# jczarnowski/DeepFactors

Hardware: NVIDIA H100
Metric: keyframe-pair Jacobian+JtJ evals/sec (640x480, C=32) (higher is better)
Workload: dtype f32

## Files before the change

### deepfactors_b200/csrc/dfk_window.cu

```cuda
#include <cuda_runtime.h>
#include <stdint.h>

#include "dfk_internal.h"

namespace dfk {

namespace {

__device__ __forceinline__ int packed_index(int i, int j, int NP) { return i * NP - (i * (i - 1)) / 2 + (j - i); }
__device__ __forceinline__ float rec_h(const float* rec, int a, int b, int NP)
{
  return a <= b ? rec[packed_index(a, b, NP)] : rec[packed_index(b, a, NP)];
}

__device__ __forceinline__ int link_row0(int r) { return r < 6 ? r : 6 + r; }
__device__ __forceinline__ int link_row1(int r, int C) { return r < 6 ? 6 + r : 6 + C + r; }

__global__ void __launch_bounds__(256)
window_assemble_kernel(WindowDev w, const float* __restrict__ records, const float* __restrict__ geo,
                       float* __restrict__ out)
{
  const int C = w.code_size, B = 6 + C, NP = 12 + C;
  const int NH = NP * (NP + 1) / 2, REC = NH + NP + 2;
  const int NG = 12 + 2 * C, NHG = NG * (NG + 1) / 2, RECG = NHG + NG + 2;
  float* tail = out + (size_t)w.num_keyframes * (B * B + B) + (size_t)w.num_pairs * B * 6;
  const int job = blockIdx.x;
  if (job < w.num_keyframes) {
    const int k = job;
    float* D = out + (size_t)k * B * B;
    float* g = out + (size_t)w.num_keyframes * B * B + (size_t)k * B;
    const int a0 = w.kf0_ptr[k], a1 = w.kf0_ptr[k + 1];
    const int b0 = w.kf1_ptr[k], b1 = w.kf1_ptr[k + 1];
    const int l00 = w.lk0_ptr[k], l01 = w.lk0_ptr[k + 1];
    const int l10 = w.lk1_ptr[k], l11 = w.lk1_ptr[k + 1];
    for (int e = threadIdx.x; e < B * B + B; e += blockDim.x) {
      float s = 0.0f;
      if (e < B * B) {
        const int r = e / B, c = e - r * B;
        const int lr = r < 6 ? r : 6 + r, lc = c < 6 ? c : 6 + c;
        for (int q = a0; q < a1; ++q) s += rec_h(records + (size_t)w.kf0_items[q] * REC, lr, lc, NP);
        if (r < 6 && c < 6)
          for (int q = b0; q < b1; ++q) s += rec_h(records + (size_t)w.kf1_items[q] * REC, 6 + r, 6 + c, NP);
        for (int q = l00; q < l01; ++q) s += rec_h(geo + (size_t)w.lk0_links[q] * RECG, link_row0(r), link_row0(c), NG);
        for (int q = l10; q < l11; ++q)
          s += rec_h(geo + (size_t)w.lk1_links[q] * RECG, link_row1(r, C), link_row1(c, C), NG);
        D[e] = s;
      } else {
        const int r = e - B * B;
        const int lr = r < 6 ? r : 6 + r;
        for (int q = a0; q < a1; ++q) s -= records[(size_t)w.kf0_items[q] * REC + NH + lr];
        if (r < 6)
          for (int q = b0; q < b1; ++q) s -= records[(size_t)w.kf1_items[q] * REC + NH + 6 + r];
        for (int q = l00; q < l01; ++q) s -= geo[(size_t)w.lk0_links[q] * RECG + NHG + link_row0(r)];
        for (int q = l10; q < l11; ++q) s -= geo[(size_t)w.lk1_links[q] * RECG + NHG + link_row1(r, C)];
        g[r] = s;
      }
    }
  } else if (job < w.num_keyframes + w.num_pairs) {
    const int p = job - w.num_keyframes;
    float* O = out + (size_t)w.num_keyframes * (B * B + B) + (size_t)p * B * 6;
    const int i0 = w.pair_ptr[p], i1 = w.pair_ptr[p + 1];
    for (int e = threadIdx.x; e < B * 6; e += blockDim.x) {
      const int r = e / 6, c = e - r * 6;
      const int lr = r < 6 ? r : 6 + r;
      float s = 0.0f;
      for (int q = i0; q < i1; ++q) s += rec_h(records + (size_t)w.pair_items[q] * REC, lr, 6 + c, NP);
      O[e] = s;
    }
  } else if (job < w.num_keyframes + w.num_pairs + w.num_links) {
    const int l = job - w.num_keyframes - w.num_pairs;
    float* O = tail + 2 + (size_t)l * B * B;
    const float* rec = geo + (size_t)l * RECG;
    for (int e = threadIdx.x; e < B * B; e += blockDim.x) {
      const int r = e / B, c = e - r * B;
      O[e] = rec_h(rec, link_row0(r), link_row1(c, C), NG);
    }
  } else {
    __shared__ float red_f[8], red_i[8];
    float f = 0.0f, ni = 0.0f;
    for (int i = threadIdx.x; i < w.num_items; i += blockDim.x) {
      const float* rec = records + (size_t)i * REC;
      const uint32_t inl = __float_as_uint(rec[NH + NP + 1]);
      if (w.item_area[i] == 0.0f) {
        f += rec[NH + NP];
      } else {
        if (inl > 0) f += rec[NH + NP] / (float)inl * w.item_area[i];
        ni += (float)inl;
      }
    }
    for (int l = threadIdx.x; l < w.num_links; l += blockDim.x) f += geo[(size_t)l * RECG + NHG + NG];
    for (int o = 16; o > 0; o >>= 1) {
      f += __shfl_xor_sync(0xffffffffu, f, o);
      ni += __shfl_xor_sync(0xffffffffu, ni, o);
    }
    if ((threadIdx.x & 31) == 0) {
      red_f[threadIdx.x >> 5] = f;
      red_i[threadIdx.x >> 5] = ni;
    }
    __syncthreads();
    if (threadIdx.x == 0) {
      float sf = 0.0f, si = 0.0f;
      for (int k = 0; k < (int)(blockDim.x >> 5); ++k) {
        sf += red_f[k];
        si += red_i[k];
      }
      tail[0] = sf;
      tail[1] = si;
    }
  }
}

}

cudaError_t launch_window_assemble(const WindowDev& w, const float* records_dev, const float* geo_records_dev,
                                   float* out_dev, cudaStream_t stream)
{
  window_assemble_kernel<<<w.num_keyframes + w.num_pairs + w.num_links + 1, 256, 0, stream>>>(w, records_dev,
                                                                                             geo_records_dev, out_dev);
  return cudaGetLastError();
}

}
```

Before: 32190.

## Split window assembly across more blocks, unroll gathers, enable programmatic dependent launch

Each keyframe, pair and link job is now spread over several blocks so every thread computes exactly one output element, instead of one block looping over all elements. The gather loops are unrolled by four so index and record loads can be issued in parallel. The kernel is launched with programmatic stream serialization and calls cudaGridDependencySynchronize, which lets its launch overlap the tail of the previous kernel. This adds blocks and some index arithmetic, and it relies on PDL support.

```diff
diff --git a/deepfactors_b200/csrc/dfk_window.cu b/deepfactors_b200/csrc/dfk_window.cu
--- a/deepfactors_b200/csrc/dfk_window.cu
+++ b/deepfactors_b200/csrc/dfk_window.cu
@@ -8,75 +8,90 @@
 namespace {
 
 __device__ __forceinline__ int packed_index(int i, int j, int NP) { return i * NP - (i * (i - 1)) / 2 + (j - i); }
-__device__ __forceinline__ float rec_h(const float* rec, int a, int b, int NP)
-{
-  return a <= b ? rec[packed_index(a, b, NP)] : rec[packed_index(b, a, NP)];
-}
 
 __device__ __forceinline__ int link_row0(int r) { return r < 6 ? r : 6 + r; }
 __device__ __forceinline__ int link_row1(int r, int C) { return r < 6 ? 6 + r : 6 + C + r; }
 
-__global__ void __launch_bounds__(256)
+constexpr int kWinThreads = 256;
+constexpr int kWinUnroll = 4;
+
+template <bool SUB>
+__device__ __forceinline__ float gather(float s, const float* __restrict__ base, size_t stride, int off,
+                                        const int* __restrict__ idx, int q0, int q1)
+{
+  for (int q = q0; q < q1; q += kWinUnroll) {
+    int id[kWinUnroll];
+#pragma unroll
+    for (int u = 0; u < kWinUnroll; ++u) id[u] = q + u < q1 ? idx[q + u] : 0;
+    float v[kWinUnroll];
+#pragma unroll
+    for (int u = 0; u < kWinUnroll; ++u) v[u] = q + u < q1 ? base[(size_t)id[u] * stride + off] : 0.0f;
+#pragma unroll
+    for (int u = 0; u < kWinUnroll; ++u)
+      if (q + u < q1) s = SUB ? s - v[u] : s + v[u];
+  }
+  return s;
+}
+
+__device__ __forceinline__ int sym_off(int a, int b, int NP) { return a <= b ? packed_index(a, b, NP) : packed_index(b, a, NP); }
+
+__global__ void __launch_bounds__(kWinThreads)
 window_assemble_kernel(WindowDev w, const float* __restrict__ records, const float* __restrict__ geo,
                        float* __restrict__ out)
 {
   const int C = w.code_size, B = 6 + C, NP = 12 + C;
   const int NH = NP * (NP + 1) / 2, REC = NH + NP + 2;
   const int NG = 12 + 2 * C, NHG = NG * (NG + 1) / 2, RECG = NHG + NG + 2;
+  const int SK = (B * B + B + kWinThreads - 1) / kWinThreads, SP = (B * 6 + kWinThreads - 1) / kWinThreads,
+            SL = (B * B + kWinThreads - 1) / kWinThreads;
+  const int JK = w.num_keyframes * SK, JP = JK + w.num_pairs * SP, JL = JP + w.num_links * SL;
   float* tail = out + (size_t)w.num_keyframes * (B * B + B) + (size_t)w.num_pairs * B * 6;
   const int job = blockIdx.x;
-  if (job < w.num_keyframes) {
-    const int k = job;
+  cudaGridDependencySynchronize();
+  if (job < JK) {
+    const int k = job / SK;
+    const int e = (job - k * SK) * kWinThreads + threadIdx.x;
+    if (e >= B * B + B) return;
     float* D = out + (size_t)k * B * B;
     float* g = out + (size_t)w.num_keyframes * B * B + (size_t)k * B;
     const int a0 = w.kf0_ptr[k], a1 = w.kf0_ptr[k + 1];
     const int b0 = w.kf1_ptr[k], b1 = w.kf1_ptr[k + 1];
     const int l00 = w.lk0_ptr[k], l01 = w.lk0_ptr[k + 1];
     const int l10 = w.lk1_ptr[k], l11 = w.lk1_ptr[k + 1];
-    for (int e = threadIdx.x; e < B * B + B; e += blockDim.x) {
-      float s = 0.0f;
-      if (e < B * B) {
-        const int r = e / B, c = e - r * B;
-        const int lr = r < 6 ? r : 6 + r, lc = c < 6 ? c : 6 + c;
-        for (int q = a0; q < a1; ++q) s += rec_h(records + (size_t)w.kf0_items[q] * REC, lr, lc, NP);
-        if (r < 6 && c < 6)
-          for (int q = b0; q < b1; ++q) s += rec_h(records + (size_t)w.kf1_items[q] * REC, 6 + r, 6 + c, NP);
-        for (int q = l00; q < l01; ++q) s += rec_h(geo + (size_t)w.lk0_links[q] * RECG, link_row0(r), link_row0(c), NG);
-        for (int q = l10; q < l11; ++q)
-          s += rec_h(geo + (size_t)w.lk1_links[q] * RECG, link_row1(r, C), link_row1(c, C), NG);
-        D[e] = s;
-      } else {
-        const int r = e - B * B;
-        const int lr = r < 6 ? r : 6 + r;
-        for (int q = a0; q < a1; ++q) s -= records[(size_t)w.kf0_items[q] * REC + NH + lr];
-        if (r < 6)
-          for (int q = b0; q < b1; ++q) s -= records[(size_t)w.kf1_items[q] * REC + NH + 6 + r];
-        for (int q = l00; q < l01; ++q) s -= geo[(size_t)w.lk0_links[q] * RECG + NHG + link_row0(r)];
-        for (int q = l10; q < l11; ++q) s -= geo[(size_t)w.lk1_links[q] * RECG + NHG + link_row1(r, C)];
-        g[r] = s;
-      }
+    float s = 0.0f;
+    if (e < B * B) {
+      const int r = e / B, c = e - r * B;
+      const int lr = r < 6 ? r : 6 + r, lc = c < 6 ? c : 6 + c;
+      s = gather<false>(s, records, REC, sym_off(lr, lc, NP), w.kf0_items, a0, a1);
+      if (r < 6 && c < 6) s = gather<false>(s, records, REC, sym_off(6 + r, 6 + c, NP), w.kf1_items, b0, b1);
+      s = gather<false>(s, geo, RECG, sym_off(link_row0(r), link_row0(c), NG), w.lk0_links, l00, l01);
+      s = gather<false>(s, geo, RECG, sym_off(link_row1(r, C), link_row1(c, C), NG), w.lk1_links, l10, l11);
+      D[e] = s;
+    } else {
+      const int r = e - B * B;
+      const int lr = r < 6 ? r : 6 + r;
+      s = gather<true>(s, records, REC, NH + lr, w.kf0_items, a0, a1);
+      if (r < 6) s = gather<true>(s, records, REC, NH + 6 + r, w.kf1_items, b0, b1);
+      s = gather<true>(s, geo, RECG, NHG + link_row0(r), w.lk0_links, l00, l01);
+      s = gather<true>(s, geo, RECG, NHG + link_row1(r, C), w.lk1_links, l10, l11);
+      g[r] = s;
     }
-  } else if (job < w.num_keyframes + w.num_pairs) {
-    const int p = job - w.num_keyframes;
+  } else if (job < JP) {
+    const int p = (job - JK) / SP;
+    const int e = (job - JK - p * SP) * kWinThreads + threadIdx.x;
+    if (e >= B * 6) return;
     float* O = out + (size_t)w.num_keyframes * (B * B + B) + (size_t)p * B * 6;
-    const int i0 = w.pair_ptr[p], i1 = w.pair_ptr[p + 1];
-    for (int e = threadIdx.x; e < B * 6; e += blockDim.x) {
-      const int r = e / 6, c = e - r * 6;
-      const int lr = r < 6 ? r : 6 + r;
-      float s = 0.0f;
-      for (int q = i0; q < i1; ++q) s += rec_h(records + (size_t)w.pair_items[q] * REC, lr, 6 + c, NP);
-      O[e] = s;
-    }
-  } else if (job < w.num_keyframes + w.num_pairs + w.num_links) {
-    const int l = job - w.num_keyframes - w.num_pairs;
-    float* O = tail + 2 + (size_t)l * B * B;
-    const float* rec = geo + (size_t)l * RECG;
-    for (int e = threadIdx.x; e < B * B; e += blockDim.x) {
-      const int r = e / B, c = e - r * B;
-      O[e] = rec_h(rec, link_row0(r), link_row1(c, C), NG);
-    }
+    const int r = e / 6, c = e - r * 6;
+    const int lr = r < 6 ? r : 6 + r;
+    O[e] = gather<false>(0.0f, records, REC, sym_off(lr, 6 + c, NP), w.pair_items, w.pair_ptr[p], w.pair_ptr[p + 1]);
+  } else if (job < JL) {
+    const int l = (job - JP) / SL;
+    const int e = (job - JP - l * SL) * kWinThreads + threadIdx.x;
+    if (e >= B * B) return;
+    const int r = e / B, c = e - r * B;
+    tail[2 + (size_t)l * B * B + e] = geo[(size_t)l * RECG + sym_off(link_row0(r), link_row1(c, C), NG)];
   } else {
-    __shared__ float red_f[8], red_i[8];
+    __shared__ float red_f[kWinThreads / 32], red_i[kWinThreads / 32];
     float f = 0.0f, ni = 0.0f;
     for (int i = threadIdx.x; i < w.num_items; i += blockDim.x) {
       const float* rec = records + (size_t)i * REC;
@@ -115,9 +130,21 @@
 cudaError_t launch_window_assemble(const WindowDev& w, const float* records_dev, const float* geo_records_dev,
                                    float* out_dev, cudaStream_t stream)
 {
-  window_assemble_kernel<<<w.num_keyframes + w.num_pairs + w.num_links + 1, 256, 0, stream>>>(w, records_dev,
-                                                                                             geo_records_dev, out_dev);
-  return cudaGetLastError();
+  const int B = 6 + w.code_size;
+  const int jobs = w.num_keyframes * ((B * B + B + kWinThreads - 1) / kWinThreads) +
+                   w.num_pairs * ((B * 6 + kWinThreads - 1) / kWinThreads) +
+                   w.num_links * ((B * B + kWinThreads - 1) / kWinThreads) + 1;
+  cudaLaunchConfig_t cfg{};
+  cfg.gridDim = dim3(jobs);
+  cfg.blockDim = dim3(kWinThreads);
+  cfg.dynamicSmemBytes = 0;
+  cfg.stream = stream;
+  cudaLaunchAttribute attr[1];
+  attr[0].id = cudaLaunchAttributeProgrammaticStreamSerialization;
+  attr[0].val.programmaticStreamSerializationAllowed = 1;
+  cfg.attrs = attr;
+  cfg.numAttrs = 1;
+  return cudaLaunchKernelEx(&cfg, window_assemble_kernel, w, records_dev, geo_records_dev, out_dev);
 }
 
 }
```

Measured after the change: 32940 (median of 6 runs). +2.3%, better.
